# KyungMinJin/OTPose

Measured on AMD Instinct MI355X. Metric: frames/sec at 384x288, 5-frame window, batch 16; heatmap max-abs delta vs ref, higher is better.
Workload: dtype f32 storage+accumulate / f16x3 split products; 1 GPU; BASELINE configs[1]: batch 16 x 5-frame x 384x288, HRNet-W48 + DCN warp + ConvVideoTransformer, fp32 forward (eval), seeded synthetic weights; clips_per_gpu=16, parallelism=dp1, outputs_finite=True

## Files before the change

### include/otpose_hip.h

```cpp
#ifndef OTPOSE_HIP_H
#define OTPOSE_HIP_H

#include <stddef.h>

#ifdef __cplusplus
extern "C" {
#endif

#define OTP_OK 0
#define OTP_ERR_BAD_ARG (-1)
#define OTP_ERR_UNSUPPORTED (-2)
#define OTP_ERR_LAUNCH (-3)
#define OTP_ERR_WORKSPACE (-4)

#define OTP_DTYPE_F32 0
#define OTP_DTYPE_F16 1
#define OTP_DTYPE_BF16 2
#define OTP_DTYPE_F64 3

#define OTP_ACT_NONE 0
#define OTP_ACT_RELU 1
#define OTP_ACT_GELU 2

int otp_version(void);
// ... 53 lines not shown
                                      int pad_w, int dil_h, int dil_w, int groups, int deformable_groups, int dtype,
                                      int has_mask);
int otp_mdcn_backward(const void* x, const void* offset, const void* mask, const void* weight,
                      const void* grad_out, void* grad_x, void* grad_offset, void* grad_mask,
                      void* grad_weight, void* grad_bias, void* workspace, size_t workspace_bytes,
                      int N, int C, int H, int W, int Cout, int kh, int kw,
                      int stride, int pad, int dil, int groups, int deformable_groups,
                      int dtype, void* stream);
int otp_mdcn_backward_ex(const void* x, const void* offset, const void* mask, const void* weight, const void* grad_out,
                         void* grad_x, void* grad_offset, void* grad_mask, void* grad_weight, void* grad_bias, void* workspace,
                         size_t workspace_bytes, int N, int C, int H, int W, int Cout, int kh, int kw, int stride_h, int stride_w,
                         int pad_h, int pad_w, int dil_h, int dil_w, int groups, int deformable_groups, int dtype, void* stream);

int otp_deform_psroi_pool_forward(const void* data, const void* rois, const void* offset, void* out, void* out_count, int N, int C,
                                  int H, int W, int num_rois, int offset_channels, int no_trans, float spatial_scale,
                                  int out_channels, int group_size, int pooled_size, int part_size, int sample_per_part,
                                  float trans_std, int dtype, void* stream);
size_t otp_deform_psroi_pool_backward_workspace(int N, int C, int H, int W, int num_rois, int offset_channels, int no_trans,
                                                int out_channels, int group_size, int pooled_size, int part_size,
                                                int sample_per_part, int dtype);
int otp_deform_psroi_pool_backward(const void* grad_out, const void* data, const void* rois, const void* offset,
                                   const void* out_count, void* grad_input, void* grad_offset, int N, int C, int H, int W,
                                   int num_rois, int offset_channels, int no_trans, float spatial_scale, int out_channels,
                                   int group_size, int pooled_size, int part_size, int sample_per_part, float trans_std,
                                   void* workspace, size_t workspace_bytes, int dtype, void* stream);

typedef struct otp_conv_desc {
    int N, Cin, H, W, Cout, kh, kw, stride, pad, dil;
    int in_ctot, in_coff, in2_ctot, in2_coff, out_ctot, out_coff;
    int res_ctot, res_coff, res_up, act, Ho, Wo, frame_split;
    float out_scale;
    int res_layout;
} otp_conv_desc;

int otp_conv2d_set_tile(int MB, int PB, int WM, int WP);
int otp_conv2d_last_plan(int* out8);
int otp_conv2d_plan(const otp_conv_desc* desc, int* out8);
int otp_conv2d_pack_weight(const void* weight, void* wpacked, int Cout, int Cin, int kh, int kw, void* stream);
int otp_conv2d(const void* in, const void* in2, const void* wpacked, const void* scale, const void* shift,
               const void* res, void* out, const otp_conv_desc* desc, void* stream);

size_t otp_conv2d_wino_weight_bytes(int Cout, int Cin);
int otp_conv2d_wino_pack_weight(const void* weight, void* upacked, int Cout, int Cin, void* stream);
int otp_conv2d_wino_supported(const otp_conv_desc* desc);
int otp_conv2d_wino_last_plan(int* out4);
int otp_conv2d_wino(const void* in, const void* upacked, const void* scale, const void* shift, const void* res, void* out,
                    const otp_conv_desc* desc, void* stream);

int otp_conv3x3_small_supported(const otp_conv_desc* desc);
size_t otp_conv3x3_small_weight_bytes(int Cout, int Cin);
int otp_conv3x3_small_pack(const void* weight, void* wpacked, int Cout, int Cin, void* stream);
int otp_conv3x3_small(const void* in, const void* in2, const void* wpacked, const void* scale, const void* shift, void* out,
                      const otp_conv_desc* desc, void* stream);

size_t otp_conv2d_x3_weight_bytes(int Cout, int Cin, int k, int stride);
int otp_conv2d_x3_pack_weight(const void* weight, const void* scale, void* wpacked, int Cout, int Cin, int k, int stride,
                              void* stream);
int otp_conv2d_x3_supported(const otp_conv_desc* desc);
int otp_conv2d_x3(const void* in, const void* wpacked, const void* shift, const void* res, void* out,
                  const otp_conv_desc* desc, void* stream);

#define OTP_S8_F32_C4 1
#define OTP_S8_F32_NCHW 2
size_t otp_s8_bytes(int N, int C, int H, int W);
int otp_s8_pack(const void* in_f32, void* out_s8, void* out_c4, int N, int C, int H, int W, int in_ctot, int in_coff, void* stream);
int otp_s8_upsample_add(const void* const* lows, const int* factors, int nlow, const void* res, void* out_nchw, void* out_s8,
                        void* out_c4, int N, int C, int Hh, int Wh, int relu, int res_ctot, int res_coff, int out_ctot,
                        int out_coff, void* stream);
int otp_s8_upsample_add_ex(const void* const* lows, const int* factors, int nlow, const void* res, int res_layout, void* out_nchw,
                           void* out_s8, void* out_c4, int N, int C, int Hh, int Wh, int relu, int res_ctot, int res_coff,
                           int out_ctot, int out_coff, void* stream);
int otp_s8_unpack(const void* in_s8, void* out_f32, int N, int C, int H, int W, void* stream);
int otp_c4_unpack(const void* in_c4, void* out_f32, int N, int C, int H, int W, void* stream);
int otp_conv3x3_s8_supported(const otp_conv_desc* desc);
size_t otp_conv3x3_s8_weight_bytes(int Cout, int Cin);
int otp_conv3x3_s8_pack_weight(const void* weight, const void* scale, void* wpacked, int Cout, int Cin, void* stream);
int otp_conv3x3_s8(const void* in_s8, const void* wpacked, const void* shift, const void* res_c4, void* out_f32,
                   int out_f32_layout, void* out_s8, const otp_conv_desc* desc, void* stream);
int otp_conv3x3_s2_s8_supported(const otp_conv_desc* desc, int nchw_out);
int otp_conv3x3_s2_s8(const void* in_s8, const void* wpacked, const void* shift, const void* res_nchw, void* out_nchw,
                      void* out_s8, const otp_conv_desc* desc, void* stream);

int otp_conv2d_pack_weight_dgrad(const void* weight, void* wpacked, int Cout, int Cin, int kh, int kw, void* stream);
int otp_dilate(const void* in, void* out, int planes, int Hi, int Wi, int s, int H, int W, void* stream);
size_t otp_conv2d_wgrad_workspace(int Cin, int Cout);
int otp_conv2d_wgrad(const void* x, const void* grad_out, void* grad_weight, int N, int Cin, int H, int W, int Cout,
                     int kh, int kw, int stride, int pad, int dil, int x_ctot, int x_coff, int dy_ctot, int dy_coff,
                     void* workspace, size_t workspace_bytes, void* stream);
size_t otp_bn_workspace(int N, int C, int HW);
int otp_bn_train_forward(const void* x, const void* gamma, const void* beta, const void* res, void* y, void* save_mean,
                         void* save_rstd, void* running_mean, void* running_var, void* workspace, size_t workspace_bytes,
                         int N, int C, int HW, float eps, float momentum, int relu, int x_ctot, int x_coff, int res_ctot,
                         int res_coff, int y_ctot, int y_coff, void* stream);
int otp_bn_train_backward(const void* grad_y, const void* x, const void* y_relu, const void* save_mean,
                          const void* save_rstd, const void* gamma, void* grad_x, void* grad_res, void* grad_gamma,
                          void* grad_beta, void* workspace, size_t workspace_bytes, int N, int C, int HW, int dy_ctot,
                          int dy_coff, int x_ctot, int x_coff, int y_ctot, int y_coff, void* stream);
int otp_channel_sum(const void* a, void* out, void* workspace, size_t workspace_bytes, int N, int C, int HW, int a_ctot,
                    int a_coff, void* stream);

int otp_dcn_fused_supported(int Cin, int J, int H, int W, int ND);
size_t otp_dcn_fused_weight_bytes(int ND, int J);
int otp_dcn_fused_pack(const void* const* w_off, const void* const* w_mask, const void* const* w_dcn, const void* const* bias,
                       void* packed, int ND, int J, void* stream);
size_t otp_dcn_fused_workspace(int B, int H, int W);
int otp_dcn_fused_forward(const void* trans, const void* x, const void* packed, void* out, void* workspace,
// ... 259 lines not shown
```

### otpose_amd/csrc/common.h

```cpp
#pragma once
#include <hip/hip_runtime.h>
#include <stddef.h>
#include <stdint.h>

#include <atomic>

#include "../../include/otpose_hip.h"

#define OTP_LDS_LIMIT (160 * 1024)

static inline int otp_launch_status() {
    return hipGetLastError() == hipSuccess ? OTP_OK : OTP_ERR_LAUNCH;
}

#define OTP_MAX_DEVICES 64
#define OTP_ALLOW_BIG_LDS(kern, bytes)                                                                      \
    do {                                                                                                    \
        if ((bytes) > 64 * 1024) {                                                                          \
            static std::atomic<uint64_t> otp_done_{0};                                                      \
            int otp_dev_ = 0;                                                                               \
            (void)hipGetDevice(&otp_dev_);                                                                  \
            const uint64_t otp_bit_ = 1ull << (otp_dev_ & (OTP_MAX_DEVICES - 1));                           \
            if (!(otp_done_.load(std::memory_order_acquire) & otp_bit_)) {                                  \
                (void)hipFuncSetAttribute(reinterpret_cast<const void*>(kern),                              \
// ... 49 lines not shown
    const otp_f32x2 t2 = t * t;
    otp_f32x2 p = t2 * -2.72614225801306e-10f + 2.77068142495902e-08f;
    p = p * t2 + -2.10102402082508e-06f;
    p = p * t2 + -5.69250639462346e-05f;
    p = p * t2 + -7.34990630326855e-04f;
    p = p * t2 + -2.95459980854025e-03f;
    p = p * t2 + -1.60960333262415e-02f;
    p = p * t;
    otp_f32x2 q = t2 * -1.45660718464996e-05f + -2.13374055278905e-04f;
    q = q * t2 + -1.68282697438203e-03f;
    q = q * t2 + -7.37332916720468e-03f;
    q = q * t2 + -1.42647390514189e-02f;
    otp_f32x2 r;
    r.x = __builtin_amdgcn_rcpf(q.x);
    r.y = __builtin_amdgcn_rcpf(q.y);
    const otp_f32x2 e = p * r, hx = x * 0.5f;
    return hx * e + hx;
}

#define OTP_BUFFER_DWORD3 0x00020000
typedef __amdgpu_buffer_rsrc_t otp_rsrc;
constexpr int OTP_OOB = -16;
__device__ __forceinline__ otp_rsrc make_rsrc(const void* p, size_t bytes) {
    return __builtin_amdgcn_make_buffer_rsrc(const_cast<void*>(p), 0,
                                             (int)(bytes > 0xffffffffull ? 0xffffffffull : bytes), OTP_BUFFER_DWORD3);
}
__device__ __forceinline__ otp_rsrc make_rsrc32(const void* p, unsigned bytes) {
    return __builtin_amdgcn_make_buffer_rsrc(const_cast<void*>(p), 0, (int)bytes, OTP_BUFFER_DWORD3);
}
__device__ __forceinline__ float bload(otp_rsrc r, int voff_bytes, int soff_bytes) {
    return __builtin_bit_cast(float, __builtin_amdgcn_raw_buffer_load_b32(r, voff_bytes, soff_bytes, 0));
}

#ifdef OTP_X3_BF16
typedef __bf16 otp_x3_t;
#define OTP_X3_MFMA __builtin_amdgcn_mfma_f32_16x16x32_bf16
#else
typedef _Float16 otp_x3_t;
#define OTP_X3_MFMA __builtin_amdgcn_mfma_f32_16x16x32_f16
#endif
typedef otp_x3_t otp_x3x2 __attribute__((ext_vector_type(2)));
typedef otp_x3_t otp_x3x8 __attribute__((ext_vector_type(8)));
__device__ __forceinline__ otp_f32x2 otp_x3_widen(uint32_t pair) {
    return __builtin_convertvector(__builtin_bit_cast(otp_x3x2, pair), otp_f32x2);
}

#ifdef OTP_X3_BF16
#define OTP_RANGE_LIMIT 3.0e38f
#else
#define OTP_RANGE_LIMIT 65504.f
#endif
enum {
    OTP_RANGE_CONVX = 1, OTP_RANGE_CONVS = 2, OTP_RANGE_CONVS2 = 3, OTP_RANGE_POINTX = 4, OTP_RANGE_STEM = 5, OTP_RANGE_S8PASS = 6,
    OTP_RANGE_MLPX = 7, OTP_RANGE_DENSEX = 8, OTP_RANGE_ATTN = 9, OTP_RANGE_DCNF = 10, OTP_RANGE_H16 = 11
};
unsigned* otp_range_word();
#ifdef OTP_NO_RANGE_GUARD
__device__ __forceinline__ bool otp_out_of_range(float) { return false; }
#else
__device__ __forceinline__ bool otp_out_of_range(float v) { return !(__builtin_fabsf(v) < OTP_RANGE_LIMIT); }
#endif
__device__ __forceinline__ void otp_range_report(unsigned* word, bool bad, unsigned code) {
    if (bad && word) __hip_atomic_store(word, code, __ATOMIC_RELAXED, __HIP_MEMORY_SCOPE_SYSTEM);
}
__device__ __forceinline__ float otp_relu(float x) {
    float y;
    asm("v_max_f32 %0, 0, %1" : "=v"(y) : "v"(x));
    return y;
}
__device__ __forceinline__ otp_f32x4 bload4(otp_rsrc r, int voff_bytes) {
    return __builtin_bit_cast(otp_f32x4, __builtin_amdgcn_raw_buffer_load_b128(r, voff_bytes, 0, 0));
}
__device__ __forceinline__ void bstore(float v, otp_rsrc r, int voff_bytes, int soff_bytes) {
    __builtin_amdgcn_raw_buffer_store_b32(__builtin_bit_cast(int, v), r, voff_bytes, soff_bytes, 0);
}

template <int NTHR, int BLKB>
__device__ __forceinline__ void otp_lds_stage(const unsigned char* __restrict__ src, unsigned char* lds) {
    constexpr int UNITS = BLKB / 16, NST = (UNITS + NTHR - 1) / NTHR;
    static_assert(BLKB % 1024 == 0, "whole wave-instructions");
    const int wave = __builtin_amdgcn_readfirstlane(threadIdx.x >> 6), lane = threadIdx.x & 63;
#pragma unroll
    for (int i = 0; i < NST; ++i) {
        const int u0 = i * NTHR + wave * 64;
        if (UNITS % NTHR != 0 && u0 * 16 >= BLKB) break;
        __builtin_amdgcn_global_load_lds((const __attribute__((address_space(1))) void*)(src + (size_t)(u0 + lane) * 16),
                                         (__attribute__((address_space(3))) void*)(lds + u0 * 16), 16, 0, 0);
    }
}
```

### otpose_amd/engine.py

```python
from __future__ import annotations

import ctypes
import dataclasses
import os
import sys
import warnings
from typing import Callable, List, Optional, Tuple

import torch

from . import hip, ops
from .ops import ACT_GELU, ACT_NONE, ACT_RELU, View

def _pair(v):
    return (int(v), int(v)) if isinstance(v, int) else (int(v[0]), int(v[1]))


def plain_conv(cv, k, stride=1, pad="same", dil=1, groups=1, bias=False, cin=None, cout=None) -> bool:
    if pad == "same":
        pad = (dil or 1) * (k // 2)
    return (cv.kernel_size == (k, k) and (stride is None or cv.stride == (stride, stride))
            and (pad is None or tuple(cv.padding) == (pad, pad)) and (dil is None or tuple(cv.dilation) == (dil, dil))
            and (groups is None or cv.groups == groups) and (bias is None or (cv.bias is not None) == bias)
            and (cin is None or cv.in_channels == cin) and (cout is None or cv.out_channels == cout))


@dataclasses.dataclass(frozen=True)
class Routes:
    use_graph: bool = True
    use_winograd: bool = True
    use_x3: bool = True
    use_dcn_fused: bool = True
    use_s8: bool = True
    use_flow_fused: bool = True
    use_small_conv: bool = True
    use_fused_mlp: bool = True
    fuse_shortcut: bool = True
    fuse_upsample: bool = True
    use_dense_cc: bool = True
    use_qkv_front: bool = True
    use_pointx: bool = True
    pointx_fuse: bool = True
    pointx_any: bool = False
    multi_stream: bool = True
    f32_tail: int = 0
    h16_tail: bool = True
    range_check: str = "defer"
    s8_residual: bool = True
    s8_lazy_nchw: bool = True
    s8_stride2: bool = True
    t1_s8: bool = True
    l1_s8: bool = True
    l1_pair: bool = True
    stem_x3: bool = True
    chain_modules: bool = True
    up_any_width: bool = True
    conv_log: bool = False
    poison: Optional[Tuple[int, int]] = None
    te_serial: bool = False

    @classmethod
    def from_env(cls) -> "Routes":
        env = os.environ.get
        on = lambda name: env("OTPOSE_" + name, "1") != "0"
        x3 = env("OTPOSE_CONV_MATH", "x3") != "f32"
        poison = env("OTPOSE_POISON")
        return cls(use_graph=on("HIP_GRAPH"), use_winograd=on("WINOGRAD"), use_x3=x3, use_dcn_fused=x3 and on("DCN_FUSED"),
                   use_s8=x3 and on("S8"), use_flow_fused=on("FLOW_FUSED"), use_small_conv=on("SMALL_CONV"),
                   use_fused_mlp=on("FUSED_MLP"), fuse_shortcut=on("FUSE_SHORTCUT"), fuse_upsample=on("FUSE_UPSAMPLE"),
                   use_dense_cc=on("DENSE_CC"), use_qkv_front=on("QKV_FRONT"), use_pointx=x3 and on("POINTX"),
                   pointx_fuse=on("POINTX_FUSE"), pointx_any=env("OTPOSE_POINTX_ANY", "0") == "1", multi_stream=on("STREAMS"),
                   f32_tail=int(env("OTPOSE_F32_TAIL", "0")) if x3 else 0, h16_tail=on("H16_TAIL"),
                   range_check=env("OTPOSE_RANGE_CHECK", "defer"), s8_residual=on("S8_RESIDUAL"), s8_lazy_nchw=on("S8_LAZY_NCHW"),
                   s8_stride2=on("S8_STRIDE2"), t1_s8=on("T1_S8"), l1_s8=on("L1_S8"), l1_pair=on("L1_PAIR"), stem_x3=on("STEM_X3"),
                   chain_modules=on("CHAIN_MODULES"), up_any_width=on("UP_ANY_WIDTH"), conv_log=bool(env("OTPOSE_CONV_LOG")),
                   poison=tuple(int(v) for v in poison.split(":")) if poison else None, te_serial=env("OTPOSE_TE_SERIAL") == "1")

    @property
    def lazy_nchw(self) -> bool:
        return self.s8_residual and self.s8_lazy_nchw


class Aux:
    __slots__ = ("s8", "c4", "nchw_needed")

    def __init__(self, s8=None, c4=None, nchw_needed=False):
        self.s8, self.c4, self.nchw_needed = s8, c4, nchw_needed


class InferenceEngine:
    h16 = False

    def __init__(self, model, batch: int, device, use_graph: bool | None = None, stream_set: int = 0, inp=None, margin=None):
        routes = Routes.from_env()
        self._init(device, routes, routes.use_graph if use_graph is None else use_graph, stream_set)
        self.B = batch
        self.model = model
        cfg = model.cfg
        self.J = model.num_joints
        self.F = getattr(model, "window_frames", 5)
        self.W_img, self.H_img = cfg.MODEL.IMAGE_SIZE
        self.h, self.w = model.pe_h, model.pe_w
        self._given = (inp, margin)
        self.param_version = self._param_version()
        with torch.no_grad():
            self._build()

    def _init(self, device, routes: Routes, use_graph: bool, stream_set: int = 0):
        device = torch.device(device)
        if device.type != "cuda" or not torch.cuda.is_available():
            raise RuntimeError("otpose_amd.OTPose runs on an MI355X through libotpose_hip.so; "
                               f"got device '{device}' (there is no CPU or PyTorch-op fallback)")
        self.lib, self.dev, self.routes = hip.lib(), device, routes
        self.model, self.B, self.inp, self.margin = None, 0, None, None
        self.ops: List[Callable] = []
        self._pair_s8 = {}
        self.l1_pairs = 0
        self._aux = {}
        self._keep = []
        self._bufs = []
        self._stream = None
        self.use_graph, self.graph = use_graph, None
        self._exact = False
        self._sid = 0
        self._side = hip.side_streams(device, 3, 4 * stream_set) if routes.multi_stream else []

    @classmethod
    def bare(cls, device, multi_stream=False):
        self = cls.__new__(cls)
# ... 79 lines not shown
        self.ops.append((run, -1))

    def on_stream(self, sid):
        self._sid = sid if (self.multi_stream and 0 <= sid <= len(self._side)) else 0

    def call(self, fn, name, *args):
        def run():
            hip.check(fn(*args, self._stream), name)
        self._emit(run)

    def call_lazy_nchw(self, aux: Aux, fn, name, args_of, unpack=None):
        full, lean = args_of(True), args_of(False)
        if unpack is None:
            def run():
                hip.check(fn(*(full if aux.nchw_needed else lean), self._stream), name)
        else:
            s8_unpack = self.lib.otp_s8_unpack

            def run():
                hip.check(fn(*lean, self._stream), name)
                if aux.nchw_needed:
                    hip.check(s8_unpack(*unpack, self._stream), "otp_s8_unpack")
        self._emit(run)

    def _bn_fold(self, bn, bias=None):
        g, b = self.dev_param(bn.weight), self.dev_param(bn.bias)
        mu, var = self.dev_param(bn.running_mean), self.dev_param(bn.running_var)
        sc = (g / torch.sqrt(var + bn.eps)).contiguous()
        sh = b - mu * sc
        if bias is not None:
            sh = sh + self.dev_param(bias) * sc
        sh = sh.contiguous()
        self._keep += [sc, sh]
        return sc, sh

    def conv(self, inp: View, weight, out: View, stride=1, pad=0, dil=1, bn=None, bias=None, act=ACT_NONE,
             res: View = None, in2: View = None, res_up=1, frame_split=0, cin=None, scale=None, shift=None):
        for v_ in (inp, in2, res):
            self._needs_nchw(v_)
        r = self.routes
        w = self.dev_param(weight)
        if w.dim() == 3:
            w = w.unsqueeze(-1)
        cout, cin_w, kh, kw = w.shape
        if bn is not None:
            sc, sh = self._bn_fold(bn, bias)
        else:
            sc = self.dev_param(scale) if scale is not None else None
            sh = shift if shift is not None else bias
            sh = self.dev_param(sh) if sh is not None else None
        d = ops.conv_desc(inp, out, cout, kh, kw, stride, pad, dil, act, in2, res, res_up, frame_split, cin)
        self._keep.append(d)
        L = self.lib
        if r.conv_log:
            route = ("x3" if r.use_x3 and in2 is None and (kh, kw) in ((3, 3), (1, 1)) and ops.x3_supported(d) else
                     "wino" if r.use_winograd and in2 is None and self.winograd_pays(cin_w, cout) and ops.wino_supported(d)
                     else "direct")
            print(f"conv {d.N}x{d.Cin}->{cout} k{kh} s{stride} p{pad} d{dil} {d.H}x{d.W} in2={in2 is not None} "
                  f"res={res is not None} up={res_up} fs={frame_split} {route}", file=sys.stderr)
        if r.use_small_conv and in2 is not None and res is None and (kh, kw) == (3, 3) and ops.small_conv_supported(d):
            wc = ops.pack_small_conv_weight(w)
            self._keep.append(wc)
            self.call(L.otp_conv3x3_small, "otp_conv3x3_small", *ops.conv3x3_small_args(inp, in2, wc, sc, sh, out, d))
            return out
        if (r.use_pointx and not self._exact and in2 is None and (kh, kw) == (1, 1) and stride == 1 and pad == 0 and res_up <= 1
                and not frame_split and act in (ACT_NONE, ACT_RELU) and inp.C == cin_w
                and (cin_w in (64, 128, 256) or (r.pointx_fuse and cin_w % 16 == 0) or r.pointx_any)
                and ops.pointwise_x3_supported(cin_w, cout, inp.t.shape[2] * inp.t.shape[3])):
            pk = ops.pack_pointwise_x3(w, sc, sh)
            self._keep.append(pk)
            self.call(L.otp_pointwise_x3, "otp_pointwise_x3", *ops.pointwise_x3_args(inp, pk, out, res, act == ACT_RELU))
            return out
        if r.use_x3 and not self._exact and in2 is None and (kh, kw) in ((3, 3), (1, 1)) and ops.x3_supported(d):
            e = ops.x3_weight_exponent(w, sc)
            d.out_scale = 2.0 ** -e
            xp = ops.pack_x3_weight(w, sc, stride, e)
            self._keep.append(xp)
            self.call(L.otp_conv2d_x3, "otp_conv2d_x3", *ops.conv2d_x3_args(inp, xp, sh, out, d, res))
            return out
        if r.use_winograd and in2 is None and self.winograd_pays(cin_w, cout) and ops.wino_supported(d):
            up = ops.pack_wino_weight(w)
            self._keep.append(up)
            self.call(L.otp_conv2d_wino, "otp_conv2d_wino", *ops.conv2d_wino_args(inp, up, sc, sh, out, d, res))
            return out
        wp = ops.pack_conv_weight(w)
        self._keep.append(wp)
        self.call(L.otp_conv2d, "otp_conv2d", *ops.conv2d_args(inp, wp, sc, sh, out, d, in2, res))
        return out

    def conv_bn(self, inp: View, conv_mod, bn_mod, act=ACT_NONE, res=None, out=None, res_up=1, **kw):
        n, _, h, w = inp.t.shape
        if kw.get("frame_split"):
            n = n * (inp.ctot // kw["cin"])
        k, s, p, dl = conv_mod.kernel_size[0], conv_mod.stride[0], conv_mod.padding[0], conv_mod.dilation[0]
        ho = (h + 2 * p - (dl * (k - 1) + 1)) // s + 1
        wo = (w + 2 * p - (dl * (k - 1) + 1)) // s + 1
        if out is None:
            f = max(res_up, 1)
            out = View(self.new(n, conv_mod.out_channels, ho * f, wo * f))
        return self.conv(inp, conv_mod.weight, out, s, p, dl, bn=bn_mod, bias=conv_mod.bias, act=act, res=res,
                         res_up=res_up, **kw)

    def dense(self, xs, packs, ress, outs, B, C, T):
        ax, ap, ar, ao = ops.dense_cc_args(xs, packs, ress, outs)
        self._keep += [ax, ap, ar, ao, *packs]
        x3 = self.use_x3 and ops.dense_x3_supported(C, T)
        fn = (self.lib.otp_dense_h1 if self.half_products else self.lib.otp_dense_x3) if x3 else self.lib.otp_dense_cc
        self.call(fn, "otp_dense_cc", ax, ap, ar, ao, len(xs), B, C, T)

    def basic_block(self, blk, x: View) -> View:
        y = self.conv_bn(x, blk.conv1, blk.bn1, ACT_RELU)
        res = x
# ... 628 lines not shown
        self.on_stream(0)
        self.fork((1,))
        self.conv_transformer(m.temporal_encoder1, x1, s1)
        final(m.final_layer1, s1, 0)
        self.on_stream(0 if self.routes.te_serial else 1)
        self.conv_transformer(m.temporal_encoder2, x2, s2)
        final(m.final_layer2, s2, 1)
        self.on_stream(0)
        self.join((1, 2))
        trans = self.rsb_chain(m.offset_mask_combine_conv, View(cat3))
        out = self.new(B, J, h, w)
        nd = len(m.deformable_conv_dilations)
        dils = [int(d) for d in m.deformable_conv_dilations]
        cin_t = trans.C
        if (self.use_dcn_fused and trans.coff == 0 and trans.C == trans.ctot and ops.dcn_fused_supported(cin_t, J, h, w, nd)
                and all(plain_conv(c[0], 3, dil=d, groups=None) for cs in (m.offsets_list, m.masks_list) for c, d in zip(cs, dils))
                and all(tuple(mm.deform_conv.weight.shape) == (J, J, 3, 3) and mm.deform_conv.deformable_groups == J
                        and mm.deform_conv.groups == 1 and _pair(mm.deform_conv.stride) == (1, 1)
                        and _pair(mm.deform_conv.padding) == (d, d) == _pair(mm.deform_conv.dilation)
                        for mm, d in zip(m.modulated_deform_conv_list, dils))):
            dcs = [mm.deform_conv for mm in m.modulated_deform_conv_list]
            packed = ops.pack_dcn_fused([self.dev_param(c[0].weight) for c in m.offsets_list],
                                        [self.dev_param(c[0].weight) for c in m.masks_list],
                                        [self.dev_param(dc.weight) for dc in dcs],
                                        [None if dc.bias is None else self.dev_param(dc.bias) for dc in dcs])
            ws = self.new(int(L.otp_dcn_fused_workspace(B, h, w)) // 4)
            dl = (ctypes.c_int * nd)(*dils)
            self._keep += [packed, dl]
            self.call(L.otp_dcn_fused_forward, "otp_dcn_fused_forward", hip.ptr(trans.t), hip.ptr(def_h.t), hip.ptr(packed),
                      hip.ptr(out), hip.ptr(ws), ws.numel() * 4, B, cin_t, J, h, w, dl, nd, 1.0 / nd)
            self._finish(out, rough, inter, prev_b, ctx, squeezed, total)
            return
        off_buf, msk_buf = self.new(B, J * 18, h, w), self.new(B, J * 9, h, w)
        for i, d in enumerate(m.deformable_conv_dilations):
            self.conv(trans, m.offsets_list[i][0].weight, View(off_buf), 1, d, d)
            self.conv(trans, m.masks_list[i][0].weight, View(msk_buf), 1, d, d)
            dc = m.modulated_deform_conv_list[i].deform_conv
            wt, bs = self.dev_param(dc.weight), self.dev_param(dc.bias)
            self.call(L.otp_mdcn_forward, "otp_mdcn_forward", hip.ptr(def_h.t), hip.ptr(off_buf), hip.ptr(msk_buf),
                      hip.ptr(wt), hip.ptr(bs), hip.ptr(out), B, J, h, w, J, 3, 3, 1, d, d, 1, J,
                      1.0 / nd, 0.0 if i == 0 else 1.0, 0)
        self._finish(out, rough, inter, prev_b, ctx, squeezed, total)

    def _finish(self, out, rough, inter, prev_b, ctx, squeezed, total):
        B, J, h, w = self.B, self.J, self.h, self.w
        if self.use_x3 or self.h16:
            self.call(self.lib.otp_range_poison, "otp_range_poison", hip.ptr(out), out.numel())
        self.outputs = (out, rough, inter, prev_b, ctx.view(B, J, h, w), squeezed, total)
        torch.cuda.synchronize(self.dev)

    _RANGE_KERNELS = {1: "convx (3x3 / 1x1 convolutions from fp32 NCHW)", 2: "convs (BasicBlock convolutions on S8 records)",
                      3: "convs2 (stride-2 convolutions on S8 records)", 4: "pointx (1x1 convolutions)", 5: "stem convolution",
                      6: "S8 conversion / fuse passes", 7: "mlpx (TransformerBlock MLP)", 8: "densex (q / k / v / proj projections)",
                      9: "channel attention", 10: "dcn_fused (warping head)", 11: "fp16 engine kernels"}

    def _raise_range(self, code):
        raise FloatingPointError(
            "otpose_amd: a value left the range of the half-precision operand pieces (|x| >= 65504, or a non-finite sum) in the "
            f"{self._RANGE_KERNELS.get(code, 'kernel family %d' % code)} of an eval forward; the heat-maps of that forward were "
            "NaN-filled on the device.  The reference computes these layers in fp32: rescale the input / check the checkpoint's "
            "BatchNorm statistics, or run the exact-fp32 kernels (OTPOSE_CONV_MATH=f32).")

    def check_range(self):
        torch.cuda.synchronize(self.dev)
        code = self.lib.otp_range_flag_read(1)
        if code:
            self._raise_range(code)

    def __del__(self):
        try:
            if getattr(self, "graph", None) is not None:
                torch.cuda.synchronize(self.dev)
        except Exception:
            pass

    def copy_into(self, src: View, dst: View):
        assert src.coff == 0 and src.C == src.ctot
        self.call(self.lib.otp_upsample_linear, "otp_upsample_linear", *ops.upsample_linear_args(src.t, dst.t, 1, dst.coff))

    def _launch_all(self, first=0, last=None):
        main = hip.stream_of(self.inp)
        handles = [main] + [s_.cuda_stream for s_ in self._side]
        for op, sid in self.ops[first:last]:
            self._stream = handles[sid] if sid > 0 else main
            op()
        self._stream = main

    def run(self, x, margin, alias_outputs: bool = False):
        if not x.is_cuda:
            raise RuntimeError("OTPose.forward expects CUDA (HIP) tensors; there is no CPU path")
        if self.range_check != "off":
            code = self.lib.otp_range_flag_read(1)
            if code:
                self._raise_range(code)
        if x.dtype == torch.uint8:
            ops.frames_to_clip(x, out=self.inp)
        elif x.data_ptr() != self.inp.data_ptr():
            self.inp.copy_(x)
        if margin.data_ptr() != self.margin.data_ptr():
            self.margin.copy_(margin.to(torch.float32))
        if self.use_graph:
            from . import parallel
            if not parallel.graph_replay_safe():
                self.use_graph = False
                self._parked_graph, self.graph = self.graph, None
        if self.use_graph and self.graph is None:
            self._launch_all()
# ... 20 lines not shown
```

### otpose_amd/ops.py

```python
from __future__ import annotations

import ctypes
import math
import os

import torch
from torch.autograd import Function

from . import hip
from .augment import FLIP_PAIRS

_K = hip.CONSTANTS
_DTYPE_F32 = _K["OTP_DTYPE_F32"]


def _require_gpu(*tensors):
    for t in tensors:
        if t is not None and not t.is_cuda:
            raise NotImplementedError("otpose_amd operators run on the GPU only (no CPU path)")


def _check_f32(*tensors):
    for t in tensors:
        if t is not None and t.dtype != torch.float32:
# ... 396 lines not shown
    wt = _image(L.otp_conv3x3_small_weight_bytes(cout, cin), torch.float32, w.device,
                ValueError, f"otp_conv3x3_small: unsupported channel counts ({cout}, {cin})")
    hip.check(L.otp_conv3x3_small_pack(hip.ptr(w), hip.ptr(wt), cout, cin, hip.stream_of(w)), "otp_conv3x3_small_pack")
    return wt


def conv3x3_small_args(inp: View, in2: View, wpacked, scale, shift, out: View, desc):
    return (_vp(inp), _vp(in2), hip.ptr(wpacked), hip.ptr(scale), hip.ptr(shift), _vp(out), desc)


def conv3x3_small(x, weight, scale=None, shift=None, act=ACT_NONE, in2=None):
    _require_gpu(x, weight)
    _check_f32(x)
    n, cin, h, w = x.shape
    cout = weight.shape[0]
    out = torch.empty(n, cout, h, w, dtype=torch.float32, device=x.device)
    iv, ov = View(x.contiguous()), View(out)
    i2 = View(in2.contiguous()) if in2 is not None else None
    d = conv_desc(iv, ov, cout, 3, 3, 1, 1, 1, act, i2)
    wt = pack_small_conv_weight(weight)
    _launch(hip.lib().otp_conv3x3_small, "otp_conv3x3_small", conv3x3_small_args(iv, i2, wt, scale, shift, ov, d), x)
    return out


def x3_weight_exponent(weight, scale=None) -> int:
    if os.environ.get("OTPOSE_X3_WSCALE", "1") == "0":
        return 0
    return h16_weight_exponent(weight, scale)


def _scaled_vec(scale, k, cout, device):
    sc = _f32(scale, device)
    if k == 0:
        return sc
    f = float(2.0 ** k)
    return sc * f if sc is not None else torch.full((cout,), f, dtype=torch.float32, device=device)


def pack_x3_weight(weight, scale=None, stride=1, k=0):
    _require_gpu(weight)
    _check_f32(weight)
    w = _f32(weight)
    if w.dim() == 3:
        w = w.unsqueeze(-1)
    cout, cin, kh, kw = w.shape
    assert kh == kw and kh in (1, 3)
    L = hip.lib()
    u = _image(L.otp_conv2d_x3_weight_bytes(cout, cin, kh, stride), torch.int32, w.device,
               ValueError, f"otp_conv2d_x3: unsupported channel counts ({cout}, {cin})")
    sc = _scaled_vec(scale, k, cout, w.device)
    hip.check(L.otp_conv2d_x3_pack_weight(hip.ptr(w), hip.ptr(sc), hip.ptr(u), cout, cin, kh, stride, hip.stream_of(w)),
              "otp_conv2d_x3_pack_weight")
    return u


def x3_supported(desc) -> bool:
    return bool(hip.lib().otp_conv2d_x3_supported(desc))


def conv2d_x3_args(inp: View, wpacked, shift, out: View, desc, res: View = None):
    return (_vp(inp), hip.ptr(wpacked), hip.ptr(shift), _vp(res), _vp(out), desc)


def conv2d_x3_launch(inp: View, wpacked, shift, out: View, desc, res: View = None, stream=None):
    _launch(hip.lib().otp_conv2d_x3, "otp_conv2d_x3", conv2d_x3_args(inp, wpacked, shift, out, desc, res), out.t, stream)


def conv2d_x3(x, weight, scale=None, shift=None, act=ACT_NONE, res=None, pad=1, dil=1, stride=1):
    _require_gpu(x, weight)
    n, cin, h, w = x.shape
    cout, k = weight.shape[0], weight.shape[2]
    ho, wo = _out_hw(h, w, k, k, stride, pad, dil)
    out = torch.empty(n, cout, ho, wo, dtype=torch.float32, device=x.device)
    iv, ov = View(x.contiguous()), View(out)
    rv = View(res.contiguous()) if res is not None else None
    d = conv_desc(iv, ov, cout, k, k, stride, pad, dil, act, None, rv)
    e = x3_weight_exponent(weight, scale)
    d.out_scale = 2.0 ** -e
    conv2d_x3_launch(iv, pack_x3_weight(weight, scale, stride, e), shift, ov, d, rv)
    return out


S8_F32_C4, S8_F32_NCHW = _K["OTP_S8_F32_C4"], _K["OTP_S8_F32_NCHW"]


def s8_empty(n, c, h, w, device):
    nbytes = hip.lib().otp_s8_bytes(n, c, h, w)
    if not nbytes:
        raise ValueError(f"S8 images need a channel count that is a multiple of 8, got {c}")
    return torch.empty(nbytes // 4, dtype=torch.int32, device=device)


def c4_empty(n, c, h, w, device):
    assert c % 4 == 0
    return torch.empty(n * c * h * w, dtype=torch.float32, device=device)


def s8_pack(inp, out=None, out_c4=None, stream=None):
    iv = inp if isinstance(inp, View) else View(inp.contiguous())
    _require_gpu(iv.t)
    n, _, h, w = iv.t.shape
    out = s8_empty(n, iv.C, h, w, iv.t.device) if out is None else out
    hip.check(hip.lib().otp_s8_pack(hip.ptr(iv.t), hip.ptr(out), hip.ptr(out_c4), n, iv.C, h, w, iv.ctot, iv.coff,
                                    stream if stream is not None else hip.stream_of(iv.t)), "otp_s8_pack")
    return out

# ... 1166 lines not shown
```

Measured before the change: 3208 frames/s.

## Add MFMA split-f16 3x3 conv kernel for small-channel convolutions

Adds a new kernel for 3x3 stride-1 convolutions with at most 32 input and output channels. It stages split hi/lo f16 weights and an input tile with halo in LDS and computes the products with three MFMA passes, optionally summing a second input. The engine routes eligible convolutions (including the in2 case previously sent to the small-conv path) to it by default. This replaces slower direct or small-conv kernels for those layers, at the cost of a split-precision approximation and an added range check.

```diff
diff --git a/include/otpose_hip.h b/include/otpose_hip.h
--- a/include/otpose_hip.h
+++ b/include/otpose_hip.h
@@ -129,6 +129,12 @@
 int otp_conv3x3_small_pack(const void* weight, void* wpacked, int Cout, int Cin, void* stream);
 int otp_conv3x3_small(const void* in, const void* in2, const void* wpacked, const void* scale, const void* shift, void* out,
                       const otp_conv_desc* desc, void* stream);
+
+int otp_conv3x3_smallx_supported(const otp_conv_desc* desc);
+size_t otp_conv3x3_smallx_weight_bytes(int Cout, int Cin);
+int otp_conv3x3_smallx_pack(const void* weight, const void* scale, void* wpacked, int Cout, int Cin, void* stream);
+int otp_conv3x3_smallx(const void* in, const void* in2, const void* wpacked, const void* shift, void* out,
+                       const otp_conv_desc* desc, void* stream);
 
 size_t otp_conv2d_x3_weight_bytes(int Cout, int Cin, int k, int stride);
 int otp_conv2d_x3_pack_weight(const void* weight, const void* scale, void* wpacked, int Cout, int Cin, int k, int stride,
diff --git a/otpose_amd/csrc/common.h b/otpose_amd/csrc/common.h
--- a/otpose_amd/csrc/common.h
+++ b/otpose_amd/csrc/common.h
@@ -125,7 +125,7 @@
 #endif
 enum {
     OTP_RANGE_CONVX = 1, OTP_RANGE_CONVS = 2, OTP_RANGE_CONVS2 = 3, OTP_RANGE_POINTX = 4, OTP_RANGE_STEM = 5, OTP_RANGE_S8PASS = 6,
-    OTP_RANGE_MLPX = 7, OTP_RANGE_DENSEX = 8, OTP_RANGE_ATTN = 9, OTP_RANGE_DCNF = 10, OTP_RANGE_H16 = 11
+    OTP_RANGE_MLPX = 7, OTP_RANGE_DENSEX = 8, OTP_RANGE_ATTN = 9, OTP_RANGE_DCNF = 10, OTP_RANGE_H16 = 11, OTP_RANGE_SMALLX = 12
 };
 unsigned* otp_range_word();
 #ifdef OTP_NO_RANGE_GUARD
diff --git a/otpose_amd/csrc/smallx.hip b/otpose_amd/csrc/smallx.hip
--- /dev/null
+++ b/otpose_amd/csrc/smallx.hip
@@ -0,0 +1,256 @@
+#include "x3.h"
+
+namespace {
+
+constexpr int SX_MT = 2;
+constexpr int SX_PIX = 64 * SX_MT;
+
+struct SxPlan {
+    int N, Cin, H, W, HW, Cout;
+    int in_ctot, in_coff, in2_ctot, in2_coff, out_ctot, out_coff, act;
+    int TW, TH, twl, LW, plane, tilesX, tilesY;
+    uint32_t mLW;
+    float post;
+    unsigned* rflag;
+};
+
+constexpr int sx_rec(int ng) { return ng * 32 + 16; }
+constexpr int sx_wbytes(int nt) { return 9 * nt * 2 * 1024; }
+
+__global__ void smallx_pack_kernel(const float* __restrict__ w, const float* __restrict__ scale, otp_u32x4* __restrict__ out, int Cout,
+                                   int Cin, int NT) {
+    const int idx = blockIdx.x * blockDim.x + threadIdx.x;
+    if (idx >= 9 * NT * 64) return;
+    const int lane = idx & 63, r = idx >> 6, t = r % NT, tap = r / NT;
+    const int cout = 16 * t + (lane & 15), ci0 = 8 * (lane >> 4);
+    float v[8];
+#pragma unroll
+    for (int j = 0; j < 8; ++j) {
+        const int ci = ci0 + j;
+        v[j] = (cout < Cout && ci < Cin) ? w[((size_t)cout * Cin + ci) * 9 + tap] * (scale ? scale[cout] : 1.f) : 0.f;
+    }
+    otp_u32x4 hi, lo;
+    otp_x3_split8(v, hi, lo);
+    const size_t o = (size_t)((tap * NT + t) * 2) * 64 + lane;
+    out[o] = hi;
+    out[o + 64] = lo;
+}
+
+template <int NG, int NT>
+__global__ __launch_bounds__(256) __attribute__((amdgpu_waves_per_eu(2, 4))) void conv3x3_smallx_kernel(
+    const float* __restrict__ in, const float* __restrict__ in2, const unsigned char* __restrict__ wpk,
+    const float* __restrict__ shift, float* __restrict__ out, const SxPlan P) {
+    constexpr int REC = sx_rec(NG), LO = NG * 16, WB = sx_wbytes(NT);
+    extern __shared__ __attribute__((aligned(16))) unsigned char smem[];
+    unsigned char* wl = smem;
+    unsigned char* tile = smem + WB;
+    const int tid = threadIdx.x, lane = tid & 63;
+    const int wave = __builtin_amdgcn_readfirstlane(tid >> 6);
+    const int i16 = lane & 15, kl = lane >> 4;
+    const int tpi = P.tilesX * P.tilesY;
+    const int n = (int)blockIdx.x / tpi, t_ = (int)blockIdx.x - n * tpi;
+    const int ty0 = (t_ / P.tilesX) * P.TH, tx0 = (t_ - (t_ / P.tilesX) * P.tilesX) * P.TW;
+
+    otp_lds_stage<256, WB>(wpk, wl);
+
+    const int py = (int)otp_magic_div((uint32_t)tid, P.mLW), px = tid - py * P.LW;
+    const int y = ty0 + py - 1, x = tx0 + px - 1;
+    const bool mine = tid < P.plane;
+    const int voff = (mine && y >= 0 && y < P.H && x >= 0 && x < P.W) ? (y * P.W + x) * 4 : OTP_OOB;
+    const size_t ib = ((size_t)n * P.in_ctot + P.in_coff) * P.HW;
+    const otp_rsrc rin = make_rsrc32(in + ib, (unsigned)(((size_t)P.N * P.in_ctot * P.HW - ib) * 4));
+    float v[NG][8];
+#pragma unroll
+    for (int g = 0; g < NG; ++g)
+#pragma unroll
+        for (int e = 0; e < 8; ++e) {
+            const int c = 8 * g + e;
+            v[g][e] = bload(rin, c < P.Cin ? voff : OTP_OOB, c * P.HW * 4);
+        }
+    if (in2) {
+        const size_t ib2 = ((size_t)n * P.in2_ctot + P.in2_coff) * P.HW;
+        const otp_rsrc rin2 = make_rsrc32(in2 + ib2, (unsigned)(((size_t)P.N * P.in2_ctot * P.HW - ib2) * 4));
+        float v2[NG][8];
+#pragma unroll
+        for (int g = 0; g < NG; ++g)
+#pragma unroll
+            for (int e = 0; e < 8; ++e) {
+                const int c = 8 * g + e;
+                v2[g][e] = bload(rin2, c < P.Cin ? voff : OTP_OOB, c * P.HW * 4);
+            }
+#pragma unroll
+        for (int g = 0; g < NG; ++g)
+#pragma unroll
+            for (int e = 0; e < 8; ++e) v[g][e] += v2[g][e];
+    }
+    if (mine) {
+        unsigned char* rec = tile + tid * REC;
+#pragma unroll
+        for (int g = 0; g < NG; ++g) {
+            otp_u32x4 hi, lo;
+            otp_x3_split8(v[g], hi, lo);
+            *reinterpret_cast<otp_u32x4*>(rec + g * 16) = hi;
+            *reinterpret_cast<otp_u32x4*>(rec + LO + g * 16) = lo;
+        }
+    }
+
+    int pb[SX_MT];
+#pragma unroll
+    for (int mt = 0; mt < SX_MT; ++mt) {
+        const int m = (wave * SX_MT + mt) * 16 + i16;
+        pb[mt] = ((m >> P.twl) * P.LW + (m & (P.TW - 1))) * REC + (kl < NG ? kl : NG - 1) * 16;
+    }
+    otp_f32x4 acc[SX_MT][NT];
+#pragma unroll
+    for (int mt = 0; mt < SX_MT; ++mt)
+#pragma unroll
+        for (int t = 0; t < NT; ++t) acc[mt][t] = (otp_f32x4){0.f, 0.f, 0.f, 0.f};
+
+    asm volatile("s_waitcnt vmcnt(0)" ::: "memory");
+    __syncthreads();
+
+#pragma unroll
+    for (int tap = 0; tap < 9; ++tap) {
+        const int toff = ((tap / 3) * P.LW + tap % 3) * REC;
+        otp_x3x8 bh[SX_MT], bl[SX_MT], ah[NT], al[NT];
+#pragma unroll
+        for (int mt = 0; mt < SX_MT; ++mt) {
+            const unsigned char* b = tile + pb[mt] + toff;
+            bh[mt] = *reinterpret_cast<const otp_x3x8*>(b);
+            bl[mt] = *reinterpret_cast<const otp_x3x8*>(b + LO);
+        }
+#pragma unroll
+        for (int t = 0; t < NT; ++t) {
+            const unsigned char* a = wl + ((tap * NT + t) * 2) * 1024 + lane * 16;
+            ah[t] = *reinterpret_cast<const otp_x3x8*>(a);
+            al[t] = *reinterpret_cast<const otp_x3x8*>(a + 1024);
+        }
+#pragma unroll
+        for (int mt = 0; mt < SX_MT; ++mt)
+#pragma unroll
+            for (int t = 0; t < NT; ++t) {
+                acc[mt][t] = OTP_X3_MFMA(al[t], bh[mt], acc[mt][t], 0, 0, 0);
+                acc[mt][t] = OTP_X3_MFMA(ah[t], bl[mt], acc[mt][t], 0, 0, 0);
+                acc[mt][t] = OTP_X3_MFMA(ah[t], bh[mt], acc[mt][t], 0, 0, 0);
+            }
+    }
+
+    float sh[NT][4];
+#pragma unroll
+    for (int t = 0; t < NT; ++t)
+#pragma unroll
+        for (int r = 0; r < 4; ++r) {
+            const int co = 16 * t + 4 * kl + r;
+            sh[t][r] = (shift && co < P.Cout) ? shift[co] : 0.f;
+        }
+    const float lo = P.act == OTP_ACT_RELU ? 0.f : -INFINITY;
+    bool bad = false;
+    float* ob = out + ((size_t)n * P.out_ctot + P.out_coff) * P.HW;
+#pragma unroll
+    for (int mt = 0; mt < SX_MT; ++mt) {
+        const int m = (wave * SX_MT + mt) * 16 + i16;
+        const int oy = ty0 + (m >> P.twl), ox = tx0 + (m & (P.TW - 1));
+        const bool live = oy < P.H && ox < P.W;
+        float* op = ob + (live ? oy * P.W + ox : 0);
+#pragma unroll
+        for (int t = 0; t < NT; ++t)
+#pragma unroll
+            for (int r = 0; r < 4; ++r) {
+                const int co = 16 * t + 4 * kl + r;
+                const float yv = acc[mt][t][r] * P.post + sh[t][r];
+                const bool st = live && co < P.Cout;
+                bad |= st && otp_out_of_range(yv);
+                if (st) op[(size_t)co * P.HW] = fmaxf(yv, lo);
+            }
+    }
+    otp_range_report(P.rflag, bad, OTP_RANGE_SMALLX);
+}
+
+bool smallx_plan(const otp_conv_desc& d, SxPlan& P) {
+    if (d.kh != 3 || d.kw != 3 || d.stride != 1 || d.pad != 1 || d.dil != 1 || d.res_up > 1 || d.frame_split > 0) return false;
+    if (d.Cin < 1 || d.Cin > 32 || d.Cout < 1 || d.Cout > 32 || d.res_ctot > 0) return false;
+    if (d.act != OTP_ACT_NONE && d.act != OTP_ACT_RELU) return false;
+    if (d.N < 1 || d.H < 1 || d.W < 1 || d.Ho != d.H || d.Wo != d.W) return false;
+    P.N = d.N; P.Cin = d.Cin; P.H = d.H; P.W = d.W; P.HW = d.H * d.W; P.Cout = d.Cout;
+    P.in_ctot = d.in_ctot; P.in_coff = d.in_coff; P.in2_ctot = d.in2_ctot; P.in2_coff = d.in2_coff;
+    P.out_ctot = d.out_ctot; P.out_coff = d.out_coff; P.act = d.act;
+    P.post = d.out_scale > 0.f ? d.out_scale : 1.f;
+    double bestu = -1.0;
+    for (int twl = 3; twl <= 5; ++twl) {
+        const int tw = 1 << twl, th = SX_PIX / tw;
+        const int tx = (d.W + tw - 1) / tw, ty = (d.H + th - 1) / th;
+        const double u = (double)d.H * d.W / ((double)tx * ty * SX_PIX);
+        if (u >= bestu - 1e-9) { bestu = u > bestu ? u : bestu; P.twl = twl; }
+    }
+    P.TW = 1 << P.twl; P.TH = SX_PIX / P.TW;
+    P.LW = P.TW + 2; P.plane = P.LW * (P.TH + 2);
+    P.tilesX = (d.W + P.TW - 1) / P.TW; P.tilesY = (d.H + P.TH - 1) / P.TH;
+    P.mLW = otp_magic((uint32_t)P.LW);
+    if (P.plane > 256) return false;
+    const long hw = (long)d.H * d.W;
+    if ((long)d.N * d.in_ctot * hw * 4 >= (1l << 31) || (long)d.N * d.out_ctot * hw * 4 >= (1l << 31)) return false;
+    if (d.in2_ctot > 0 && (long)d.N * d.in2_ctot * hw * 4 >= (1l << 31)) return false;
+    return (long)d.N * P.tilesX * P.tilesY < (1l << 31);
+}
+
+template <int NG, int NT>
+int smallx_launch(const float* in, const float* in2, const unsigned char* wpk, const float* shift, float* out, const SxPlan& P,
+                  hipStream_t st) {
+    auto kern = conv3x3_smallx_kernel<NG, NT>;
+    const size_t lds = (size_t)sx_wbytes(NT) + (size_t)P.plane * sx_rec(NG);
+    OTP_ALLOW_BIG_LDS(kern, lds);
+    hipLaunchKernelGGL(kern, dim3((unsigned)(P.N * P.tilesX * P.tilesY)), dim3(256), lds, st, in, in2, wpk, shift, out, P);
+    return otp_launch_status();
+}
+
+template <int NT>
+int smallx_dispatch(const float* in, const float* in2, const unsigned char* wpk, const float* shift, float* out, const SxPlan& P,
+                    hipStream_t st) {
+    switch ((P.Cin + 7) / 8) {
+        case 1: return smallx_launch<1, NT>(in, in2, wpk, shift, out, P, st);
+        case 2: return smallx_launch<2, NT>(in, in2, wpk, shift, out, P, st);
+        case 3: return smallx_launch<3, NT>(in, in2, wpk, shift, out, P, st);
+        default: return smallx_launch<4, NT>(in, in2, wpk, shift, out, P, st);
+    }
+}
+
+}
+
+extern "C" int otp_conv3x3_smallx_supported(const otp_conv_desc* desc) {
+    if (!desc) return 0;
+    SxPlan P{};
+    return smallx_plan(*desc, P) ? 1 : 0;
+}
+
+extern "C" size_t otp_conv3x3_smallx_weight_bytes(int Cout, int Cin) {
+    if (Cout < 1 || Cout > 32 || Cin < 1 || Cin > 32) return 0;
+    return (size_t)sx_wbytes((Cout + 15) / 16);
+}
+
+extern "C" int otp_conv3x3_smallx_pack(const void* weight, const void* scale, void* wpacked, int Cout, int Cin, void* stream) {
+    if (!weight || !wpacked) return OTP_ERR_BAD_ARG;
+    if (!otp_conv3x3_smallx_weight_bytes(Cout, Cin)) return OTP_ERR_UNSUPPORTED;
+    const int NT = (Cout + 15) / 16;
+    hipLaunchKernelGGL(smallx_pack_kernel, dim3(otp_ceil_div(9 * NT * 64, 256)), dim3(256), 0, static_cast<hipStream_t>(stream),
+                       static_cast<const float*>(weight), static_cast<const float*>(scale), static_cast<otp_u32x4*>(wpacked), Cout,
+                       Cin, NT);
+    return otp_launch_status();
+}
+
+extern "C" int otp_conv3x3_smallx(const void* in, const void* in2, const void* wpacked, const void* shift, void* out,
+                                  const otp_conv_desc* desc, void* stream) {
+    if (!in || !wpacked || !out || !desc) return OTP_ERR_BAD_ARG;
+    const otp_conv_desc& d = *desc;
+    if (d.N <= 0 || d.H <= 0 || d.W <= 0) return OTP_ERR_BAD_ARG;
+    if (d.in_ctot < d.in_coff + d.Cin || d.out_ctot < d.out_coff + d.Cout || (in2 && d.in2_ctot < d.in2_coff + d.Cin))
+        return OTP_ERR_BAD_ARG;
+    if (reinterpret_cast<uintptr_t>(wpacked) & 15) return OTP_ERR_UNSUPPORTED;
+    SxPlan P{};
+    if (!smallx_plan(d, P)) return OTP_ERR_UNSUPPORTED;
+    P.rflag = otp_range_word();
+    auto st = static_cast<hipStream_t>(stream);
+    auto fi = static_cast<const float*>(in), f2 = static_cast<const float*>(in2), fh = static_cast<const float*>(shift);
+    auto fw = static_cast<const unsigned char*>(wpacked);
+    auto fo = static_cast<float*>(out);
+    return d.Cout <= 16 ? smallx_dispatch<1>(fi, f2, fw, fh, fo, P, st) : smallx_dispatch<2>(fi, f2, fw, fh, fo, P, st);
+}
diff --git a/otpose_amd/engine.py b/otpose_amd/engine.py
--- a/otpose_amd/engine.py
+++ b/otpose_amd/engine.py
@@ -58,6 +58,7 @@
     conv_log: bool = False
     poison: Optional[Tuple[int, int]] = None
     te_serial: bool = False
+    small_x3: dataclasses.InitVar[bool] = True
 
     @classmethod
     def from_env(cls) -> "Routes":
@@ -74,7 +75,15 @@
                    range_check=env("OTPOSE_RANGE_CHECK", "defer"), s8_residual=on("S8_RESIDUAL"), s8_lazy_nchw=on("S8_LAZY_NCHW"),
                    s8_stride2=on("S8_STRIDE2"), t1_s8=on("T1_S8"), l1_s8=on("L1_S8"), l1_pair=on("L1_PAIR"), stem_x3=on("STEM_X3"),
                    chain_modules=on("CHAIN_MODULES"), up_any_width=on("UP_ANY_WIDTH"), conv_log=bool(env("OTPOSE_CONV_LOG")),
-                   poison=tuple(int(v) for v in poison.split(":")) if poison else None, te_serial=env("OTPOSE_TE_SERIAL") == "1")
+                   poison=tuple(int(v) for v in poison.split(":")) if poison else None, te_serial=env("OTPOSE_TE_SERIAL") == "1",
+                   small_x3=on("SMALL_X3"))
+
+    def __post_init__(self, small_x3):
+        object.__setattr__(self, "small_x3", bool(small_x3))
+
+    @property
+    def use_small_x3(self) -> bool:
+        return self.use_x3 and self.small_x3
 
     @property
     def lazy_nchw(self) -> bool:
@@ -260,12 +269,23 @@
         d = ops.conv_desc(inp, out, cout, kh, kw, stride, pad, dil, act, in2, res, res_up, frame_split, cin)
         self._keep.append(d)
         L = self.lib
+        smallx = (r.use_small_x3 and not self._exact and res is None and (kh, kw) == (3, 3) and stride == 1 and pad == 1 and dil == 1
+                  and ops.smallx_supported(d) and not (in2 is None and ops.x3_supported(d)))
         if r.conv_log:
-            route = ("x3" if r.use_x3 and in2 is None and (kh, kw) in ((3, 3), (1, 1)) and ops.x3_supported(d) else
+            route = ("smallx" if smallx else "small" if r.use_small_conv and in2 is not None and res is None and (kh, kw) == (3, 3)
+                     and ops.small_conv_supported(d) else
+                     "x3" if r.use_x3 and in2 is None and (kh, kw) in ((3, 3), (1, 1)) and ops.x3_supported(d) else
                      "wino" if r.use_winograd and in2 is None and self.winograd_pays(cin_w, cout) and ops.wino_supported(d)
                      else "direct")
             print(f"conv {d.N}x{d.Cin}->{cout} k{kh} s{stride} p{pad} d{dil} {d.H}x{d.W} in2={in2 is not None} "
                   f"res={res is not None} up={res_up} fs={frame_split} {route}", file=sys.stderr)
+        if smallx:
+            e = ops.x3_weight_exponent(w, sc)
+            d.out_scale = 2.0 ** -e
+            xp = ops.pack_smallx_weight(w, sc, e)
+            self._keep.append(xp)
+            self.call(L.otp_conv3x3_smallx, "otp_conv3x3_smallx", *ops.conv3x3_smallx_args(inp, in2, xp, sh, out, d))
+            return out
         if r.use_small_conv and in2 is not None and res is None and (kh, kw) == (3, 3) and ops.small_conv_supported(d):
             wc = ops.pack_small_conv_weight(w)
             self._keep.append(wc)
@@ -1000,7 +1020,8 @@
     _RANGE_KERNELS = {1: "convx (3x3 / 1x1 convolutions from fp32 NCHW)", 2: "convs (BasicBlock convolutions on S8 records)",
                       3: "convs2 (stride-2 convolutions on S8 records)", 4: "pointx (1x1 convolutions)", 5: "stem convolution",
                       6: "S8 conversion / fuse passes", 7: "mlpx (TransformerBlock MLP)", 8: "densex (q / k / v / proj projections)",
-                      9: "channel attention", 10: "dcn_fused (warping head)", 11: "fp16 engine kernels"}
+                      9: "channel attention", 10: "dcn_fused (warping head)", 11: "fp16 engine kernels",
+                      12: "smallx (3x3 convolutions of at most 32 channels)"}
 
     def _raise_range(self, code):
         raise FloatingPointError(
diff --git a/otpose_amd/ops.py b/otpose_amd/ops.py
--- a/otpose_amd/ops.py
+++ b/otpose_amd/ops.py
@@ -472,6 +472,46 @@
     hip.check(L.otp_conv2d_x3_pack_weight(hip.ptr(w), hip.ptr(sc), hip.ptr(u), cout, cin, kh, stride, hip.stream_of(w)),
               "otp_conv2d_x3_pack_weight")
     return u
+
+
+def smallx_supported(desc) -> bool:
+    return bool(hip.lib().otp_conv3x3_smallx_supported(desc))
+
+
+def pack_smallx_weight(weight, scale=None, k=0):
+    _require_gpu(weight)
+    _check_f32(weight)
+    w = _f32(weight)
+    cout, cin = w.shape[:2]
+    assert tuple(w.shape[2:]) == (3, 3)
+    L = hip.lib()
+    u = _image(L.otp_conv3x3_smallx_weight_bytes(cout, cin), torch.int32, w.device,
+               ValueError, f"otp_conv3x3_smallx: unsupported channel counts ({cout}, {cin})")
+    sc = _scaled_vec(scale, k, cout, w.device)
+    hip.check(L.otp_conv3x3_smallx_pack(hip.ptr(w), hip.ptr(sc), hip.ptr(u), cout, cin, hip.stream_of(w)),
+              "otp_conv3x3_smallx_pack")
+    return u
+
+
+def conv3x3_smallx_args(inp: View, in2: View, wpacked, shift, out: View, desc):
+    return (_vp(inp), _vp(in2), hip.ptr(wpacked), hip.ptr(shift), _vp(out), desc)
+
+
+def conv3x3_smallx(x, weight, scale=None, shift=None, act=ACT_NONE, in2=None):
+    _require_gpu(x, weight)
+    _check_f32(x)
+    n, cin, h, w = x.shape
+    cout = weight.shape[0]
+    out = torch.empty(n, cout, h, w, dtype=torch.float32, device=x.device)
+    iv, ov = View(x.contiguous()), View(out)
+    i2 = View(in2.contiguous()) if in2 is not None else None
+    d = conv_desc(iv, ov, cout, 3, 3, 1, 1, 1, act, i2)
+    e = x3_weight_exponent(weight, scale)
+    d.out_scale = 2.0 ** -e
+    sh = _f32(shift, x.device)
+    wp = pack_smallx_weight(weight, scale, e)
+    _launch(hip.lib().otp_conv3x3_smallx, "otp_conv3x3_smallx", conv3x3_smallx_args(iv, i2, wp, sh, ov, d), x)
+    return out
 
 
 def x3_supported(desc) -> bool:
```

New measurement: 3236 frames/s, median of 6. No clear change (+0.9%).
